# DeepGraphLearning/ULTRA

Hardware: AMD Instinct MI355X
Metric: triples scored/sec (all-tail ranking) on FB15k237 (higher is better)
Workload: dtype f32

## Files before the change

### include/ultra_nbfnet.h

```cpp
#ifndef ULTRA_NBFNET_H
#define ULTRA_NBFNET_H

#include <stdint.h>

#ifdef __cplusplus
extern "C" {
#endif

#define ULTRA_CONV_LAYER_NORM 1
#define ULTRA_CONV_RELU 2
#define ULTRA_CONV_RESIDUAL 4
#define ULTRA_LAYER0_MAX 8
#define ULTRA_LAYER0_ONLY_FILL 16
#define ULTRA_LAYER0_SKIP_FILL 32

int32_t ultra_conv_update(const void *x, const void *agg, const void *weight, const void *bias, const void *ln_weight,
                          const void *ln_bias, void *out, int64_t rows, int32_t input_dim, int32_t output_dim, float eps,
                          int32_t flags, void *stream);

int64_t ultra_conv_update_backward_workspace(int64_t rows);
int32_t ultra_conv_update_backward(const void *x, const void *agg, const void *grad_out, const void *weight, const void *bias,
                                   const void *ln_weight, const void *ln_bias, void *grad_x, void *grad_agg, void *grad_weight,
                                   void *grad_bias, void *grad_ln_weight, void *grad_ln_bias, void *workspace,
                                   int64_t workspace_bytes, int64_t rows, int32_t input_dim, int32_t output_dim, float eps,
                                   int32_t flags, void *stream);

int32_t ultra_readout(const void *hidden, const int64_t *t_index, const void *w1, const void *query, const void *b1,
                      const void *w2, const void *b2, const int32_t *order_dev, int64_t order_len, void *score, int64_t batch,
                      int64_t num_node, int64_t n_cand, int32_t hidden_dim, int32_t feature_dim, void *stream);

int32_t ultra_batch_prologue(const int64_t *triples, int64_t batch, int64_t n_cand, int64_t num_direct_rel, int64_t *h0,
                             int64_t *r0, int32_t *side, int32_t *valid, int64_t *rel_first, void *stream);
int32_t ultra_batch_prologue_rows(const int64_t *triples, int64_t batch, int64_t n_cand, int64_t num_direct_rel, int64_t *h0,
                                  int64_t *r0, int32_t *side, int32_t *valid, int64_t *rel_first, int64_t *cand, void *stream);
int32_t ultra_readout_batch(const void *hidden, const int64_t *triples, const int32_t *side, const void *w1, const void *query,
                            const void *b1, const void *w2, const void *b2, const int32_t *order_dev, int64_t order_len,
                            void *score, int64_t batch, int64_t num_node, int64_t n_cand, int32_t hidden_dim,
                            int32_t feature_dim, void *stream);

int32_t ultra_onehot_rows(void *out, const int64_t *rows, const void *values, int64_t batch, int64_t num_node, int64_t dim,
                          void *stream);

int32_t ultra_edge_keep_mask(const int64_t *head, const int64_t *tail, const int64_t *type, int64_t num_edge,
                             const int64_t *easy_key_sorted, int64_t n_easy, int64_t num_node, int64_t num_rel, void *keep,
                             void *stream);
int32_t ultra_easy_edge_keep(const int64_t *head, const int64_t *tail, const int64_t *type, int64_t num_edge, const int64_t *h,
                             const int64_t *t, const int64_t *r, int64_t n_triple, int64_t stride, int64_t num_node,
                             int64_t num_rel, int64_t inverse_offset, void *keep, void *stream);
int32_t ultra_leave_one_out_keep(const int64_t *head, const int64_t *tail, const int64_t *type, int64_t num_edge, const int64_t *h,
                                 const int64_t *t, const int64_t *r, int64_t n_sample, int64_t stride, int64_t num_node,
                                 int64_t num_rel, int64_t inverse_offset, void *keep, int64_t keep_stride, void *stream);
int64_t ultra_easy_edge_keep_table_workspace(int64_t n_triple);
int32_t ultra_easy_edge_keep_table(const int64_t *head, const int64_t *tail, const int64_t *type, int64_t num_edge,
                                   const int64_t *h, const int64_t *t, const int64_t *r, int64_t n_triple, int64_t stride,
                                   int64_t num_node, int64_t num_rel, int64_t inverse_offset, void *workspace,
                                   int64_t workspace_bytes, void *keep, void *stream);

int32_t ultra_query_boundary(void *out, void *query_out, const int64_t *rows, const void *table, const int64_t *pick,
                             int64_t batch, int64_t num_node, int64_t table_rows, int64_t dim, const void *w1, const void *b1,
                             void *qbias_out, void *stream);

int32_t ultra_relation_projection(const void *x, const void *w0, const void *b0, const void *w2, const void *b2, void *out,
                                  int64_t rows, int32_t n_layer, int32_t dim, void *stream);

int32_t ultra_relation_projection_layers(const void *x, const void *const *w0, const void *const *b0, const void *const *w2,
                                         const void *const *b2, void *out, int64_t rows, int32_t n_layer, int32_t dim, void *stream);

int64_t ultra_relation_projection_backward_workspace(int64_t rows, int32_t n_layer);
int32_t ultra_relation_projection_backward(const void *x, const void *const *w0, const void *const *b0, const void *const *w2,
                                           const void *const *grad_out, void *grad_x, void *grad_w0, void *grad_b0, void *grad_w2,
                                           void *grad_b2, void *workspace, int64_t workspace_bytes, int64_t rows, int32_t n_layer,
                                           int32_t dim, void *stream);

int32_t ultra_filtered_rank(const void *score, const int64_t *pos_index, const int64_t *known_ptr,
                            const int64_t *known_index, int64_t batch, int64_t n_cand, int64_t *rank_out,
                            int64_t *num_negative_out, void *stream);
int32_t ultra_filtered_rank_live(const void *score, const int64_t *pos_index, const int64_t *known_ptr,
                                 const int64_t *known_index, int64_t batch, int64_t n_cand, int64_t *rank_out,
                                 int64_t *num_negative_out, const int64_t *n_live, void *stream);

int32_t ultra_strict_negatives(const int64_t *sorted_keys_dev, int64_t n_key, const int64_t *anchor_dev, const int64_t *relation_dev,
                               const int64_t *positive_dev, const void *rand_dev, int64_t n_query, int64_t n_draw, int64_t num_node,
                               int64_t num_relation, int64_t *out_dev, void *stream);

int32_t ultra_ranking_loss(const void *pred, int64_t rows, int64_t n, float temperature, float uniform_weight, void *loss,
                           void *grad, void *stream);

int32_t ultra_readout_train_forward(const void *hid, const void *query, const void *w1, const void *b1, const void *w2,
                                    const void *b2, void *h, void *score, int64_t batch, int64_t n, void *stream);
int64_t ultra_readout_train_backward_workspace(int64_t batch, int64_t n);
int32_t ultra_readout_train_backward(const void *grad_score, const void *h, const void *hid, const void *query, const void *w1,
                                     const void *w2, void *grad_hid, void *grad_query, void *grad_w1, void *grad_b1, void *grad_w2,
                                     void *grad_b2, void *work, int64_t work_bytes, int64_t batch, int64_t n, void *stream);

int32_t ultra_relation_graph_bits(const int64_t *edge_index_dev, const int64_t *edge_type_dev, int64_t num_edge, int64_t num_node,
                                  int64_t num_relation, void *hbits_dev, void *tbits_dev, void *adj_dev, int64_t *row_counts_dev,
                                  void *stream);
int32_t ultra_relation_graph_emit(const void *adj_dev, const int64_t *row_offsets_dev, int64_t num_relation, int64_t total_edges,
                                  int64_t *edge_index_out_dev, int64_t *edge_type_out_dev, void *stream);
int32_t ultra_relation_graph_dense_adjacency(const void *adj_dev, int64_t num_relation, void *a_ex_out_dev, void *stream);
int32_t ultra_relation_graph_bits_keep(const int64_t *edge_index_dev, const int64_t *edge_type_dev, const float *keep_dev,
                                       int64_t num_edge, int64_t num_node, int64_t num_relation, void *hbits_dev, void *tbits_dev,
                                       void *adj_dev, int64_t *row_counts_dev, void *stream);
int32_t ultra_relation_graph_edge_keep(const void *adj_dev, int64_t num_relation, const int64_t *rel_edge_index_dev,
                                       const int64_t *rel_edge_type_dev, int64_t num_rel_edge, float *keep_out_dev, void *stream);
int32_t ultra_relation_graph_add_edges(const int64_t *edge_index_dev, const int64_t *edge_type_dev, int64_t num_edge, int64_t num_node,
                                       int64_t num_relation, void *hbits_dev, void *tbits_dev, void *adj_dev, int64_t *row_counts_dev,
                                       int32_t *changed_dev, void *stream);

#define ULTRA_BEAM_MAX 64
#define ULTRA_BEAM_HUB_DEGREE 256
int32_t ultra_beam_search_layer(const int64_t *row_ptr, const int32_t *csr_src, const int32_t *csr_type, const int32_t *csr_eid,
                                const int64_t *hub_rows, int64_t num_hub, int64_t num_node, int64_t num_edge,
                                const void *edge_grad, const void *dist_in, int64_t tail, int32_t num_beam, void *dist_out,
                                int64_t *back_edge_out, void *stream);

int32_t ultra_beam_search_layer_batch(const int64_t *row_ptr, const int32_t *csr_src, const int32_t *csr_type,
                                      const int32_t *csr_eid, const int64_t *hub_rows, int64_t num_hub, int64_t num_node,
                                      int64_t num_edge, int64_t num_sample, const void *edge_grad, const void *dist_in,
                                      const int64_t *tails, int32_t num_beam, void *dist_out, int64_t *back_edge_out,
                                      void *stream);

#define ULTRA_RANKING_LDS_ANSWERS 2048
int32_t ultra_symbolic_traversal(const int64_t *row_ptr, const int32_t *csr_src, const int32_t *csr_type, int64_t num_node,
                                 const int64_t *r_index, int64_t batch, int32_t dtype, const void *h, void *t, void *stream);
int32_t ultra_symbolic_traversal_keep(const int64_t *row_ptr, const int32_t *csr_src, const int32_t *csr_type,
                                      const float *keep_slot, int64_t num_node, const int64_t *r_index, int64_t batch, int32_t dtype,
                                      const void *h, void *t, void *stream);
int32_t ultra_answer_ranking(const void *pred, const uint8_t *keep, const int64_t *answers, const int64_t *ans_ptr,
                             const int64_t *hard_ptr, const int64_t *num_easy, const int64_t *ws_off, void *ws, int64_t batch,
                             int64_t num_node, int64_t *answer_ranking, int64_t *ranking, void *stream);

typedef struct {
    const int32_t *row_dev, *count_dev;
    const int32_t *add_ptr_dev, *add_src_dev, *add_type_dev;
    const int32_t *dead_ptr_dev, *dead_src_dev, *dead_type_dev;
    int64_t capacity_rows, capacity_edges, capacity_keys;
} ultra_traversal_edits;
int32_t ultra_symbolic_traversal_edit_rows(const int64_t *row_ptr, const int32_t *csr_src, const int32_t *csr_type,
                                           int64_t num_node, const ultra_traversal_edits *edits, const int64_t *r_index,
                                           int64_t batch, int32_t dtype, const void *h, void *t, void *stream);

int64_t ultra_traversal_dropout_mask_words(int64_t batch);
int32_t ultra_traversal_dropout(const int64_t *edge_index, const int64_t *edge_type, int64_t num_edge, int64_t num_node,
                                int64_t num_relation, int32_t inverse_rel_plus_one, const int32_t *deg_out, const int32_t *deg_in,
                                const int64_t *r_index, int64_t batch, int32_t dtype, const void *sym, const float *q,
                                const float *u1, const float *u2, float more_dropout, void *masks, float *keep, int32_t *k_out,
                                void *stream);
int32_t ultra_query_loss(const void *pred, const uint8_t *target, int64_t rows, int64_t n, float temperature, void *work,
                         void *loss, void *grad, void *stream);

#define ULTRA_TOPK_MAX 256
#define ULTRA_TOPK_CHUNK 4096
int64_t ultra_filtered_topk_workspace(int64_t batch, int64_t n_cand, int32_t k);
int32_t ultra_filtered_topk(const void *score, const int64_t *known_ptr, const int64_t *known_index, int64_t batch,
                            int64_t n_cand, int32_t k, int64_t *ids_out, void *scores_out, int64_t *count_out, void *workspace,
                            int64_t workspace_bytes, void *stream);
int32_t ultra_filtered_topk_live(const void *score, const int64_t *known_ptr, const int64_t *known_index, int64_t batch,
                                 int64_t n_cand, int32_t k, int64_t *ids_out, void *scores_out, int64_t *count_out,
                                 void *workspace, int64_t workspace_bytes, const int64_t *n_live, void *stream);

int32_t ultra_query_segment(const int32_t *entry_depth, const int32_t *push_row, const int32_t *pop_row, const int32_t *op_ptr,
                            const int32_t *ops, int64_t batch, int64_t num_node, int32_t stack_depth, int32_t dtype,
                            int32_t logic, void *stack, const void *push_src, int64_t push_rows, void *pop_dst,
                            int64_t pop_rows, void *sym_stack, const void *sym_push_src, void *sym_pop_dst, void *stream);
int32_t ultra_nonzero_lists(const void *x, int64_t batch, int64_t n, int64_t *counts, int64_t *ptr_out, int64_t *index_out,
                            int64_t capacity, void *stream);
int32_t ultra_nonzero_lists_live(const void *x, int64_t batch, int64_t n, int64_t *counts, int64_t *ptr_out,
                                 int64_t *index_out, int64_t capacity, const int64_t *n_live, void *stream);

int64_t ultra_filtered_above_workspace(int64_t batch, int64_t n_cand);
int32_t ultra_filtered_above(const void *score, const int64_t *known_ptr, const int64_t *known_index, int64_t batch,
                             int64_t n_cand, float threshold, int64_t *ptr_out, int64_t *ids_out, void *scores_out,
                             int64_t capacity, int64_t *size_out, void *workspace, int64_t workspace_bytes, void *stream);
int32_t ultra_filtered_above_live(const void *score, const int64_t *known_ptr, const int64_t *known_index, int64_t batch,
                                  int64_t n_cand, float threshold, int64_t *ptr_out, int64_t *ids_out, void *scores_out,
                                  int64_t capacity, int64_t *size_out, void *workspace, int64_t workspace_bytes,
                                  const int64_t *n_live, void *stream);

#ifdef __cplusplus
}
#endif
#endif
```

### ultra_amd/csrc/dense_kernels.hip

```cpp
#include <hip/hip_runtime.h>

#include <cstdint>
#include <cstdio>
#include <cstdlib>
#include <string>

#include "../../include/ultra_rspmm.h"
#include "plan.hpp"
#include "device_scope.hpp"
#include "torch_math.hpp"
#include "update_tile.hpp"

namespace ultra {

#ifndef ULTRA_CONV_DEBUG
#define ULTRA_CONV_DEBUG 0
#endif
constexpr int CONV_DBG_BITS = ULTRA_CONV_DEBUG ? CONV_DBG_NO_MATRIX : 0;

struct ConvParams {
    const float *x;
    const float *agg;
    const float *weight;
    const float *bias, *ln_w, *ln_b;
    float *out;
    long long rows;
    float eps;
    int flags;
};

__global__ void __launch_bounds__(512, 2) conv_update_kernel(const ConvParams p) {
    __shared__ __attribute__((aligned(16))) float lds_w[2 * 16 * 64 * 4];
    __shared__ float lds_vec[3 * 64];
    const int tid = threadIdx.x;
    for (int idx4 = tid; idx4 < 2 * 16 * 64; idx4 += blockDim.x) {
        const int l = idx4 & 63, i = (idx4 >> 6) & 15, m = idx4 >> 10;
        const float *wr = p.weight + (32 * m + (l & 31)) * 128 + 8 * i;
        const float4 w0 = *reinterpret_cast<const float4 *>(wr), w1 = *reinterpret_cast<const float4 *>(wr + 4);
        const bool odd = (l >> 5) != 0;
        reinterpret_cast<float4 *>(lds_w)[idx4] =
            make_float4(odd ? w0.y : w0.x, odd ? w1.y : w1.x, odd ? w0.w : w0.z, odd ? w1.w : w1.z);
    }
    if (tid < 64) {
        lds_vec[tid] = p.bias ? p.bias[tid] : 0.f;
        lds_vec[64 + tid] = (p.flags & CONV_LN) ? p.ln_w[tid] : 1.f;
        lds_vec[128 + tid] = (p.flags & CONV_LN) ? p.ln_b[tid] : 0.f;
    }
    __syncthreads();
    const int lane = tid & 63, wave = tid >> 6;
    const int j = lane & 31, h = lane >> 5;
    const float4 *w4 = reinterpret_cast<const float4 *>(lds_w);
    const long long ntile = (p.rows + 31) / 32;
    const int wpb = blockDim.x >> 6;
    const long long tstride = (long long)gridDim.x * wpb;
    long long tile = (long long)blockIdx.x * wpb + wave;
    float4 bx[8], ba[8];
    if (tile < ntile) {
        const long long r0 = tile * 32 + j;
        const long long rc0 = r0 < p.rows ? r0 : p.rows - 1;
        const float4 *xr = reinterpret_cast<const float4 *>(p.x + rc0 * 64);
        const float4 *ar = reinterpret_cast<const float4 *>(p.agg + rc0 * 64);
#pragma unroll
        for (int i = 0; i < 8; ++i) bx[i] = xr[2 * i + h];
#pragma unroll
        for (int i = 0; i < 8; ++i) ba[i] = ar[2 * i + h];
    }
    for (; tile < ntile; tile += tstride) {
        const long long row = tile * 32 + j;
        const bool valid = row < p.rows;
        float4 bxn[8], ban[8];
        {
            const long long tn = tile + tstride;
            const long long rn = (tn < ntile ? tn : tile) * 32 + j;
            const long long rcn = rn < p.rows ? rn : p.rows - 1;
            const float4 *xr = reinterpret_cast<const float4 *>(p.x + rcn * 64);
            const float4 *ar = reinterpret_cast<const float4 *>(p.agg + rcn * 64);
#pragma unroll
            for (int i = 0; i < 8; ++i) bxn[i] = xr[2 * i + h];
#pragma unroll
            for (int i = 0; i < 8; ++i) ban[i] = ar[2 * i + h];
        }
        f32x16 acc0, acc1;
#pragma unroll
        for (int r = 0; r < 16; ++r) {
            acc0[r] = 0.f;
            acc1[r] = 0.f;
        }
        float4 a0 = w4[(0 * 16 + 0) * 64 + lane];
        float4 a1 = w4[(1 * 16 + 0) * 64 + lane];
        float4 bs[16];
#pragma unroll
        for (int i = 0; i < 16; ++i) {
            bs[i] = i < 8 ? bx[i] : ba[i - 8];
            swap32(bs[i].x, bs[i].y);
            swap32(bs[i].z, bs[i].w);
        }
        __builtin_amdgcn_sched_barrier(0);
        if (!(p.flags & CONV_DBG_BITS & CONV_DBG_NO_MATRIX))
#pragma unroll
        for (int i = 0; i < 16; ++i) {
            const float4 b = bs[i];
            float4 a0n = a0, a1n = a1;
            if (i + 1 < 16) {
                a0n = w4[(0 * 16 + i + 1) * 64 + lane];
                a1n = w4[(1 * 16 + i + 1) * 64 + lane];
            }
            acc0 = __builtin_amdgcn_mfma_f32_32x32x2f32(a0.x, b.x, acc0, 0, 0, 0);
            acc1 = __builtin_amdgcn_mfma_f32_32x32x2f32(a1.x, b.x, acc1, 0, 0, 0);
            acc0 = __builtin_amdgcn_mfma_f32_32x32x2f32(a0.z, b.z, acc0, 0, 0, 0);
            acc1 = __builtin_amdgcn_mfma_f32_32x32x2f32(a1.z, b.z, acc1, 0, 0, 0);
            acc0 = __builtin_amdgcn_mfma_f32_32x32x2f32(a0.y, b.y, acc0, 0, 0, 0);
            acc1 = __builtin_amdgcn_mfma_f32_32x32x2f32(a1.y, b.y, acc1, 0, 0, 0);
            acc0 = __builtin_amdgcn_mfma_f32_32x32x2f32(a0.w, b.w, acc0, 0, 0, 0);
            acc1 = __builtin_amdgcn_mfma_f32_32x32x2f32(a1.w, b.w, acc1, 0, 0, 0);
            a0 = a0n;
            a1 = a1n;
            __builtin_amdgcn_sched_barrier(0);
        }
        float v[2][16];
#pragma unroll
        for (int r = 0; r < 16; ++r) {
            v[0][r] = acc0[r] + lds_vec[feat_of(0, r, h)];
            v[1][r] = acc1[r] + lds_vec[feat_of(1, r, h)];
        }
        if (p.flags & CONV_LN) {
            float mean, rstd;
            row_moments_pair(v, h, p.eps, mean, rstd);
#pragma unroll
            for (int m = 0; m < 2; ++m)
#pragma unroll
                for (int r = 0; r < 16; ++r) {
                    const int f = feat_of(m, r, h);
                    v[m][r] = ln_apply(v[m][r], mean, rstd, lds_vec[64 + f], lds_vec[128 + f]);
                }
        }
#pragma unroll
        for (int m = 0; m < 2; ++m)
#pragma unroll
            for (int g = 0; g < 4; ++g) {
                float4 y = make_float4(v[m][4 * g + 0], v[m][4 * g + 1], v[m][4 * g + 2], v[m][4 * g + 3]);
                if (p.flags & CONV_RELU) {
                    y.x = fmaxf(y.x, 0.f);
                    y.y = fmaxf(y.y, 0.f);
                    y.z = fmaxf(y.z, 0.f);
                    y.w = fmaxf(y.w, 0.f);
                }
                if (p.flags & CONV_RESIDUAL) {
                    const float4 xi = bx[4 * m + g];
                    y.x += xi.x;
                    y.y += xi.y;
                    y.z += xi.z;
                    y.w += xi.w;
                }
                if (valid) *reinterpret_cast<float4 *>(p.out + row * 64 + 32 * m + 8 * g + 4 * h) = y;
            }
#pragma unroll
        for (int i = 0; i < 8; ++i) {
            bx[i] = bxn[i];
            ba[i] = ban[i];
        }
    }
}

struct ReadoutParams {
    const float *hidden;
    const int64_t *t_index;
    const int64_t *triples;
    const int32_t *side;
    const float *w1;
    const float *query;
    const float *b1;
    const float *w2;
    const float *b2;
    const int32_t *order;
    int order_len;
    float *score;
    long long batch, num_node, n_cand;
};

constexpr int READOUT_ORDER_MAX = 640;
constexpr int READOUT_HID_STRIDE = 132;

__device__ __forceinline__ long long readout_node(const ReadoutParams &p, const long long row, const long long b, const long long c) {
    long long node = c;
    if (p.triples)
        node = p.triples[row * 3 + (p.side[b] ? 1 : 0)];
    else if (p.t_index)
        node = p.t_index[row];
    return (node >= 0 && node < p.num_node) ? node : -1;
}

__global__ void __launch_bounds__(512) readout_kernel(const ReadoutParams p) {
    __shared__ __attribute__((aligned(16))) float lds_w[4 * 16 * 64 * 4];
    __shared__ __attribute__((aligned(16))) float lds_hid[8][16 * READOUT_HID_STRIDE];
    __shared__ float lds_lane[8][16 * 16];
    __shared__ __attribute__((aligned(16))) float lds_w2[136], lds_b1[128];
    __shared__ __attribute__((aligned(16))) int lds_order[READOUT_ORDER_MAX];
    const int tid = threadIdx.x;
    for (int idx4 = tid; idx4 < 4 * 16 * 64; idx4 += blockDim.x) {
        const int l = idx4 & 63, i = (idx4 >> 6) & 15, m = idx4 >> 10;
        const float *wr = p.w1 + (32 * m + (l & 31)) * 128 + 8 * i;
        const float4 w0 = *reinterpret_cast<const float4 *>(wr), w1 = *reinterpret_cast<const float4 *>(wr + 4);
        const bool odd = (l >> 5) != 0;
        reinterpret_cast<float4 *>(lds_w)[idx4] =
            make_float4(odd ? w0.y : w0.x, odd ? w1.y : w1.x, odd ? w0.w : w0.z, odd ? w1.w : w1.z);
    }
    if (tid < 136) lds_w2[tid] = tid < 128 ? p.w2[tid] : 0.f;
    if (tid < 128) lds_b1[tid] = p.b1[tid];
    if (p.order) {
        for (int i = tid; i < p.order_len; i += blockDim.x) lds_order[i] = p.order[i];
    } else {
        for (int i = tid; i < 8 + 128; i += blockDim.x)
            lds_order[i] = i >= 8 ? i - 8 : (i == 0 || i == 1 ? 1 : (i == 3 ? 8 : (i == 4 ? 16 : 0)));
    }
    __syncthreads();
    const int lane = tid & 63, wave = tid >> 6;
    const int j = lane & 31, h = lane >> 5;
    const float4 *w4 = reinterpret_cast<const float4 *>(lds_w);
    float *hid = lds_hid[wave];
    float *lv = lds_lane[wave];
    const long long total = p.batch * p.n_cand;
    const long long ntile = (total + 31) / 32;
    const int wpb = blockDim.x >> 6;
    const auto load_tile = [&](const long long tile, float4 (&bh)[8], float4 (&bq)[8]) {
        const long long row = tile * 32 + j;
        const long long rowc = row < total ? row : total - 1;
        const long long b = rowc / p.n_cand;
        const long long c = rowc - b * p.n_cand;
        const long long node = readout_node(p, rowc, b, c) < 0 ? 0 : readout_node(p, rowc, b, c);
        const float4 *hr = reinterpret_cast<const float4 *>(p.hidden + (b * p.num_node + node) * 64);
#pragma unroll
        for (int i = 0; i < 8; ++i) bh[i] = hr[2 * i + h];
        const float *qr = p.query + b * 64 + h;
#pragma unroll
        for (int i = 0; i < 8; ++i) bq[i] = make_float4(qr[8 * i], qr[8 * i + 4], qr[8 * i + 2], qr[8 * i + 6]);
    };
    const long long tstride = (long long)gridDim.x * wpb;
    long long tile = (long long)blockIdx.x * wpb + wave;
    float4 bh[8], bq[8];
    if (tile < ntile) load_tile(tile, bh, bq);
    for (; tile < ntile; tile += tstride) {
        float4 bhn[8], bqn[8];
        load_tile(tile + tstride < ntile ? tile + tstride : tile, bhn, bqn);
        f32x16 acc[4];
#pragma unroll
        for (int m = 0; m < 4; ++m)
#pragma unroll
            for (int r = 0; r < 16; ++r) acc[m][r] = 0.f;
        float4 a[4];
#pragma unroll
        for (int m = 0; m < 4; ++m) a[m] = w4[(m * 16 + 0) * 64 + lane];
#pragma unroll
        for (int i = 0; i < 16; ++i) {
            float4 bb;
            if (i < 8) {
                bb = bh[i];
                swap32(bb.x, bb.y);
                swap32(bb.z, bb.w);
            } else {
                bb = bq[i - 8];
            }
            float4 an[4];
#pragma unroll
            for (int m = 0; m < 4; ++m) an[m] = (i + 1 < 16) ? w4[(m * 16 + i + 1) * 64 + lane] : a[m];
#pragma unroll
            for (int m = 0; m < 4; ++m) acc[m] = __builtin_amdgcn_mfma_f32_32x32x2f32(a[m].x, bb.x, acc[m], 0, 0, 0);
#pragma unroll
            for (int m = 0; m < 4; ++m) acc[m] = __builtin_amdgcn_mfma_f32_32x32x2f32(a[m].z, bb.z, acc[m], 0, 0, 0);
#pragma unroll
            for (int m = 0; m < 4; ++m) acc[m] = __builtin_amdgcn_mfma_f32_32x32x2f32(a[m].y, bb.y, acc[m], 0, 0, 0);
#pragma unroll
            for (int m = 0; m < 4; ++m) acc[m] = __builtin_amdgcn_mfma_f32_32x32x2f32(a[m].w, bb.w, acc[m], 0, 0, 0);
#pragma unroll
            for (int m = 0; m < 4; ++m) a[m] = an[m];
            __builtin_amdgcn_sched_barrier(0);
        }
#pragma unroll 1
        for (int pass = 0; pass < 2; ++pass) {
            if ((j >> 4) == pass) {
                const int jr = j & 15;
#pragma unroll
                for (int m = 0; m < 4; ++m)
#pragma unroll
                    for (int g = 0; g < 4; ++g) {
                        const int f = feat_of(m, 4 * g, h);
                        const float4 bb = *reinterpret_cast<const float4 *>(lds_b1 + f);
                        *reinterpret_cast<float4 *>(hid + jr * READOUT_HID_STRIDE + f) =
                            make_float4(fmaxf(acc[m][4 * g + 0] + bb.x, 0.f), fmaxf(acc[m][4 * g + 1] + bb.y, 0.f),
                                        fmaxf(acc[m][4 * g + 2] + bb.z, 0.f), fmaxf(acc[m][4 * g + 3] + bb.w, 0.f));
                    }
                if (h == 0) hid[jr * READOUT_HID_STRIDE + 128] = 0.f;
            }
            __builtin_amdgcn_fence(__ATOMIC_RELEASE, "wavefront");
            __builtin_amdgcn_wave_barrier();
            __builtin_amdgcn_fence(__ATOMIC_ACQUIRE, "wavefront");
            const int pr = lane & 15, sub = lane >> 4;
            const float *hrow = hid + pr * READOUT_HID_STRIDE;
            int hdr = 1;
            float s = 0.f;
            const int n_stage = lds_order[0];
            for (int st = 0; st < n_stage; ++st) {
                const int L = lds_order[hdr], carry = lds_order[hdr + 1];
                for (int q = sub; q < L; q += 4) {
                    const int off = lds_order[hdr + 2 + 2 * q], groups = lds_order[hdr + 3 + 2 * q];
                    float v = (q == 0 && carry) ? s : 0.f;
                    for (int g = 0; g < groups; ++g) {
                        const int4 w0 = *reinterpret_cast<const int4 *>(lds_order + off + 8 * g);
                        const int4 w1 = *reinterpret_cast<const int4 *>(lds_order + off + 8 * g + 4);
                        const int word[8] = {w0.x, w0.y, w0.z, w0.w, w1.x, w1.y, w1.z, w1.w};
                        float hv[8], wv[8];
#pragma unroll
                        for (int e = 0; e < 8; ++e) {
                            hv[e] = hrow[word[e] & 255];
                            wv[e] = lds_w2[word[e] & 255];
                        }
#pragma unroll
                        for (int e = 0; e < 8; ++e)
                            v = (word[e] & 256) ? v + hv[e] * wv[e] : __builtin_fmaf(hv[e], wv[e], v);
                    }
                    lv[q * 16 + pr] = v;
                }
                __builtin_amdgcn_fence(__ATOMIC_RELEASE, "wavefront");
                __builtin_amdgcn_wave_barrier();
                __builtin_amdgcn_fence(__ATOMIC_ACQUIRE, "wavefront");
                if (sub == 0) {
                    for (int half = L >> 1; half >= 1; half >>= 1)
                        for (int q = 0; q < half; ++q) lv[q * 16 + pr] = lv[q * 16 + pr] + lv[(q + half) * 16 + pr];
                    s = lv[pr];
                }
                hdr += 2 + 2 * L;
            }
            const long long prow = tile * 32 + 16 * pass + pr;
            if (sub == 0 && prow < total) {
                const long long pb = prow / p.n_cand;
                p.score[prow] = readout_node(p, prow, pb, prow - pb * p.n_cand) < 0 ? __builtin_nanf("") : s + p.b2[0];
            }
            __builtin_amdgcn_fence(__ATOMIC_RELEASE, "wavefront");
            __builtin_amdgcn_wave_barrier();
            __builtin_amdgcn_fence(__ATOMIC_ACQUIRE, "wavefront");
        }
#pragma unroll
        for (int i = 0; i < 8; ++i) {
            bh[i] = bhn[i];
            bq[i] = bqn[i];
        }
    }
}

constexpr int RELPROJ_MAX_LAYERS = 8;
struct RelProjParams {
    const float *x;
    const float *w0[RELPROJ_MAX_LAYERS], *b0[RELPROJ_MAX_LAYERS];
    const float *w2[RELPROJ_MAX_LAYERS], *b2[RELPROJ_MAX_LAYERS];
    float *out;
    long long rows;
    int n_layer;
};

constexpr int RELPROJ_TILES = 4;

__global__ void __launch_bounds__(256) relation_projection_kernel(const RelProjParams p) {
    constexpr int STRIDE = 68;
    __shared__ __attribute__((aligned(16))) float x_lds[RELPROJ_TILES][16 * STRIDE];
    __shared__ __attribute__((aligned(16))) float h_lds[RELPROJ_TILES][16 * STRIDE];
    using f32x4 = float __attribute__((ext_vector_type(4)));
    const int tid = threadIdx.x, lane = tid & 63, wave = tid >> 6;
    const int i16 = lane & 15, kk = lane >> 4;
    const int layer = blockIdx.y;
    const long long row_base = (long long)blockIdx.x * (16 * RELPROJ_TILES);
    const float *w0 = p.w0[layer], *w2 = p.w2[layer];
#pragma unroll
    for (int t = 0; t < RELPROJ_TILES; ++t) {
        const long long row = min(row_base + 16 * t + (tid >> 4), p.rows - 1);
        *reinterpret_cast<float4 *>(x_lds[t] + (tid >> 4) * STRIDE + 4 * (tid & 15)) =
            *reinterpret_cast<const float4 *>(p.x + row * 64 + 4 * (tid & 15));
    }
    float a0[16], a2[16];
    {
        const float4 *r0 = reinterpret_cast<const float4 *>(w0 + (16 * wave + i16) * 64);
        const float4 *r2 = reinterpret_cast<const float4 *>(w2 + (16 * wave + i16) * 64);
#pragma unroll
        for (int s = 0; s < 16; ++s) {
            const float4 v0 = r0[s], v2 = r2[s];
            a0[s] = kk == 0 ? v0.x : (kk == 1 ? v0.y : (kk == 2 ? v0.z : v0.w));
            a2[s] = kk == 0 ? v2.x : (kk == 1 ? v2.y : (kk == 2 ? v2.z : v2.w));
        }
    }
    const int f0 = 16 * wave + 4 * kk;
    float b0v[4], b2v[4];
#pragma unroll
    for (int r = 0; r < 4; ++r) {
        b0v[r] = p.b0[layer][f0 + r];
        b2v[r] = p.b2[layer][f0 + r];
    }
    __syncthreads();
    f32x4 d[RELPROJ_TILES];
#pragma unroll
    for (int t = 0; t < RELPROJ_TILES; ++t)
#pragma unroll
        for (int r = 0; r < 4; ++r) d[t][r] = 0.f;
#pragma unroll
    for (int s = 0; s < 16; ++s)
#pragma unroll
        for (int t = 0; t < RELPROJ_TILES; ++t)
            d[t] = __builtin_amdgcn_mfma_f32_16x16x4f32(a0[s], x_lds[t][i16 * STRIDE + 4 * s + kk], d[t], 0, 0, 0);
#pragma unroll
    for (int t = 0; t < RELPROJ_TILES; ++t)
#pragma unroll
        for (int r = 0; r < 4; ++r) h_lds[t][i16 * STRIDE + f0 + r] = fmaxf(d[t][r] + b0v[r], 0.f);
    __syncthreads();
#pragma unroll
    for (int t = 0; t < RELPROJ_TILES; ++t)
#pragma unroll
        for (int r = 0; r < 4; ++r) d[t][r] = 0.f;
#pragma unroll
    for (int s = 0; s < 16; ++s)
#pragma unroll
        for (int t = 0; t < RELPROJ_TILES; ++t)
            d[t] = __builtin_amdgcn_mfma_f32_16x16x4f32(a2[s], h_lds[t][i16 * STRIDE + 4 * s + kk], d[t], 0, 0, 0);
#pragma unroll
    for (int t = 0; t < RELPROJ_TILES; ++t) {
        const long long row = row_base + 16 * t + i16;
        if (row < p.rows)
            *reinterpret_cast<float4 *>(p.out + ((size_t)layer * p.rows + row) * 64 + f0) =
                make_float4(d[t][0] + b2v[0], d[t][1] + b2v[1], d[t][2] + b2v[2], d[t][3] + b2v[3]);
    }
}

static int grid_for(long long ntile, int waves_per_block, int blocks_per_cu = 2) {
    static int cu = 0;
    if (cu == 0) {
        int dev = 0, v = 0;
        cu = 256;
        if (hipGetDevice(&dev) == hipSuccess &&
            hipDeviceGetAttribute(&v, hipDeviceAttributeMultiprocessorCount, dev) == hipSuccess && v > 0)
            cu = v;
    }
    long long blocks = (ntile + waves_per_block - 1) / waves_per_block;
    const long long cap = (long long)cu * blocks_per_cu;
    if (blocks > cap) blocks = cap;
    if (blocks < 1) blocks = 1;
    return (int)blocks;
}

}

using namespace ultra;

extern "C" {

int32_t ultra_conv_update(const void *x, const void *agg, const void *weight, const void *bias, const void *ln_weight,
                          const void *ln_bias, void *out, int64_t rows, int32_t input_dim, int32_t output_dim, float eps,
                          int32_t flags, void *stream) {
    ULTRA_DEVICE_SCOPE(stream, x);
    if (input_dim != 64 || output_dim != 64) {
        set_error("ultra_conv_update: only input_dim = output_dim = 64 is built (the ULTRA checkpoints' shape)");
        return ULTRA_ERR_UNSUPPORTED;
    }
    if (!x || !agg || !weight || !out || rows < 0 || ((flags & CONV_LN) && (!ln_weight || !ln_bias))) {
        set_error("ultra_conv_update: NULL operand");
        return ULTRA_ERR_INVALID;
    }
    if (flags & ~(CONV_LN | CONV_RELU | CONV_RESIDUAL | CONV_DBG_BITS)) {
        set_error("ultra_conv_update: unknown flag bits " + std::to_string(flags & ~(CONV_LN | CONV_RELU | CONV_RESIDUAL | CONV_DBG_BITS)) +
                  " (CONV_DBG_NO_MATRIX exists only in a -DULTRA_CONV_DEBUG=1 build)");
        return ULTRA_ERR_INVALID;
    }
    if (rows == 0) return ULTRA_OK;
    ConvParams p;
    p.x = (const float *)x;
    p.agg = (const float *)agg;
    p.weight = (const float *)weight;
    p.bias = (const float *)bias;
    p.ln_w = (const float *)ln_weight;
    p.ln_b = (const float *)ln_bias;
    p.out = (float *)out;
    p.rows = rows;
    p.eps = eps;
    p.flags = flags;
    const long long ntile = (rows + 31) / 32;
    int threads = ntile >= 2048 ? 512 : 256;
    int grid = grid_for(ntile, threads / 64, threads == 512 ? 1 : 2);
    {
        static int env_threads = -1, env_grid = 0;
        if (env_threads < 0) {
            env_threads = 0;
            const char *env = std::getenv("ULTRA_CONV_GEOMETRY");
            if (env && std::sscanf(env, "%d,%d", &env_threads, &env_grid) != 2) env_threads = 0;
        }
        if (env_threads > 0 && env_grid > 0) threads = env_threads, grid = env_grid;
    }
    (void)hipGetLastError();
    hipLaunchKernelGGL(conv_update_kernel, dim3(grid), dim3(threads), 0, reinterpret_cast<hipStream_t>(stream), p);
    hipError_t e = hipGetLastError();
    if (e != hipSuccess) {
        set_error(std::string("conv_update_kernel launch: ") + hipGetErrorString(e));
        return ULTRA_ERR_HIP;
    }
    return ULTRA_OK;
}

static int launch_readout(ReadoutParams &p, const void *hidden, const void *w1, const void *query, const void *b1,
                          const void *w2, const void *b2, const int32_t *order, int64_t order_len, void *score, int64_t batch,
                          int64_t num_node, int64_t n_cand, int32_t hidden_dim, int32_t feature_dim, void *stream, const char *who) {
    if (hidden_dim != 64 || feature_dim != 128) {
        set_error(std::string(who) + ": only hidden_dim = 64, feature_dim = 128 is built (the ULTRA checkpoints' shape)");
        return ULTRA_ERR_UNSUPPORTED;
    }
    if (!hidden || !w1 || !query || !b1 || !w2 || !b2 || !score || batch < 0 || n_cand < 0) {
        set_error(std::string(who) + ": NULL operand");
        return ULTRA_ERR_INVALID;
    }
    if (order && (order_len < 5 || order_len > READOUT_ORDER_MAX)) {
        set_error(std::string(who) + ": summation program longer than 640 words (or empty)");
        return ULTRA_ERR_INVALID;
    }
    if (batch * n_cand == 0) return ULTRA_OK;
    p.hidden = (const float *)hidden;
    p.w1 = (const float *)w1;
    p.query = (const float *)query;
    p.b1 = (const float *)b1;
    p.w2 = (const float *)w2;
    p.b2 = (const float *)b2;
    p.order = order;
    p.order_len = (int)order_len;
    p.score = (float *)score;
    p.batch = batch;
    p.num_node = num_node;
    p.n_cand = n_cand;
    const long long ntile = (batch * n_cand + 31) / 32;
    const int grid = grid_for(ntile, 8, 1);
    (void)hipGetLastError();
    hipLaunchKernelGGL(readout_kernel, dim3(grid), dim3(512), 0, reinterpret_cast<hipStream_t>(stream), p);
    hipError_t e = hipGetLastError();
    if (e != hipSuccess) {
        set_error(std::string("readout_kernel launch: ") + hipGetErrorString(e));
        return ULTRA_ERR_HIP;
    }
    return ULTRA_OK;
}

int32_t ultra_readout(const void *hidden, const int64_t *t_index, const void *w1, const void *query, const void *b1,
                      const void *w2, const void *b2, const int32_t *order_dev, int64_t order_len, void *score, int64_t batch,
                      int64_t num_node, int64_t n_cand, int32_t hidden_dim, int32_t feature_dim, void *stream) {
    ULTRA_DEVICE_SCOPE(stream, hidden);
    ReadoutParams p;
    p.t_index = t_index;
    p.triples = nullptr;
    p.side = nullptr;
    return launch_readout(p, hidden, w1, query, b1, w2, b2, order_dev, order_len, score, batch, num_node, n_cand, hidden_dim,
                          feature_dim, stream, "ultra_readout");
}

int32_t ultra_readout_batch(const void *hidden, const int64_t *triples, const int32_t *side, const void *w1, const void *query,
                            const void *b1, const void *w2, const void *b2, const int32_t *order_dev, int64_t order_len,
                            void *score, int64_t batch, int64_t num_node, int64_t n_cand, int32_t hidden_dim,
                            int32_t feature_dim, void *stream) {
    ULTRA_DEVICE_SCOPE(stream, hidden);
    if (!triples || !side) {
        set_error("ultra_readout_batch: NULL operand");
        return ULTRA_ERR_INVALID;
    }
    ReadoutParams p;
    p.t_index = nullptr;
    p.triples = triples;
    p.side = side;
    return launch_readout(p, hidden, w1, query, b1, w2, b2, order_dev, order_len, score, batch, num_node, n_cand, hidden_dim,
                          feature_dim, stream, "ultra_readout_batch");
}

static int32_t launch_relation_projection(RelProjParams &p, void *stream) {
    const dim3 grid((unsigned)((p.rows + 16 * RELPROJ_TILES - 1) / (16 * RELPROJ_TILES)), (unsigned)p.n_layer);
    (void)hipGetLastError();
    hipLaunchKernelGGL(relation_projection_kernel, grid, dim3(256), 0, reinterpret_cast<hipStream_t>(stream), p);
    hipError_t e = hipGetLastError();
    if (e != hipSuccess) {
        set_error(std::string("relation_projection_kernel launch: ") + hipGetErrorString(e));
        return ULTRA_ERR_HIP;
    }
    return ULTRA_OK;
}

int32_t ultra_relation_projection(const void *x, const void *w0, const void *b0, const void *w2, const void *b2, void *out,
                                  int64_t rows, int32_t n_layer, int32_t dim, void *stream) {
    ULTRA_DEVICE_SCOPE(stream, x);
    if (dim != 64 || n_layer > RELPROJ_MAX_LAYERS) {
        set_error("ultra_relation_projection: only dim = 64 and at most 8 layers are built (the ULTRA checkpoints' shape)");
        return ULTRA_ERR_UNSUPPORTED;
    }
    if (!x || !w0 || !b0 || !w2 || !b2 || !out || rows < 0 || n_layer < 0) {
        set_error("ultra_relation_projection: NULL operand");
        return ULTRA_ERR_INVALID;
    }
    if (rows == 0 || n_layer == 0) return ULTRA_OK;
    RelProjParams p;
    p.x = (const float *)x;
    for (int l = 0; l < n_layer; ++l) {
        p.w0[l] = (const float *)w0 + (size_t)l * 64 * 64, p.b0[l] = (const float *)b0 + (size_t)l * 64;
        p.w2[l] = (const float *)w2 + (size_t)l * 64 * 64, p.b2[l] = (const float *)b2 + (size_t)l * 64;
    }
    p.out = (float *)out;
    p.rows = rows;
    p.n_layer = n_layer;
    return launch_relation_projection(p, stream);
}

int32_t ultra_relation_projection_layers(const void *x, const void *const *w0, const void *const *b0, const void *const *w2,
                                         const void *const *b2, void *out, int64_t rows, int32_t n_layer, int32_t dim,
                                         void *stream) {
    ULTRA_DEVICE_SCOPE(stream, x);
    if (dim != 64 || n_layer > RELPROJ_MAX_LAYERS) {
        set_error("ultra_relation_projection_layers: only dim = 64 and at most 8 layers are built (the ULTRA checkpoints' shape)");
        return ULTRA_ERR_UNSUPPORTED;
    }
    if (!x || !w0 || !b0 || !w2 || !b2 || !out || rows < 0 || n_layer < 0) {
        set_error("ultra_relation_projection_layers: NULL operand");
        return ULTRA_ERR_INVALID;
    }
    if (rows == 0 || n_layer == 0) return ULTRA_OK;
    RelProjParams p;
    p.x = (const float *)x;
    for (int l = 0; l < n_layer; ++l) {
        if (!w0[l] || !b0[l] || !w2[l] || !b2[l]) {
            set_error("ultra_relation_projection_layers: NULL layer parameter");
            return ULTRA_ERR_INVALID;
        }
        p.w0[l] = (const float *)w0[l], p.b0[l] = (const float *)b0[l], p.w2[l] = (const float *)w2[l], p.b2[l] = (const float *)b2[l];
    }
    p.out = (float *)out;
    p.rows = rows;
    p.n_layer = n_layer;
    return launch_relation_projection(p, stream);
}

}
```

Measured before the change: 212.5 million.

## Restructure readout kernel scheduling, prefetch, and precomputed walk coefficients with tracing hooks

Each wave now takes a contiguous range of tiles instead of a grid stride, and the first tile's hidden rows are prefetched before the weight staging so the global loads overlap setup. Two register buffers ping-pong between tiles, with incremental batch and candidate indices replacing per-tile divisions. The bias and ReLU move out of the per-pass store loop. The summation walk reads precomputed w2 coefficients and byte offsets, with a fast path when a group has no rounded elements. Invalid-node flags come from registers via shuffle instead of re-reading the triples. It also adds clock64 tracing and an env-var grid override, which cost only a pointer check when off, but the extra buffers raise register and LDS pressure.

```diff
diff --git a/include/ultra_nbfnet.h b/include/ultra_nbfnet.h
--- a/include/ultra_nbfnet.h
+++ b/include/ultra_nbfnet.h
@@ -37,6 +37,7 @@
                             const void *b1, const void *w2, const void *b2, const int32_t *order_dev, int64_t order_len,
                             void *score, int64_t batch, int64_t num_node, int64_t n_cand, int32_t hidden_dim,
                             int32_t feature_dim, void *stream);
+int32_t ultra_readout_trace(void *trace_dev);
 
 int32_t ultra_onehot_rows(void *out, const int64_t *rows, const void *values, int64_t batch, int64_t num_node, int64_t dim,
                           void *stream);
diff --git a/ultra_amd/csrc/dense_kernels.hip b/ultra_amd/csrc/dense_kernels.hip
--- a/ultra_amd/csrc/dense_kernels.hip
+++ b/ultra_amd/csrc/dense_kernels.hip
@@ -176,9 +176,11 @@
     int order_len;
     float *score;
     long long batch, num_node, n_cand;
+    long long *trace;
 };
 
 constexpr int READOUT_ORDER_MAX = 640;
+constexpr int READOUT_ELEM_OFFSET = 0x3fc, READOUT_ELEM_ROUNDED = 1 << 11, READOUT_ELEM_GROUP_ROUNDED = 1 << 12;
 constexpr int READOUT_HID_STRIDE = 132;
 
 __device__ __forceinline__ long long readout_node(const ReadoutParams &p, const long long row, const long long b, const long long c) {
@@ -194,54 +196,82 @@
     __shared__ __attribute__((aligned(16))) float lds_w[4 * 16 * 64 * 4];
     __shared__ __attribute__((aligned(16))) float lds_hid[8][16 * READOUT_HID_STRIDE];
     __shared__ float lds_lane[8][16 * 16];
-    __shared__ __attribute__((aligned(16))) float lds_w2[136], lds_b1[128];
+    __shared__ __attribute__((aligned(16))) float lds_w2p[READOUT_ORDER_MAX], lds_b1[128], lds_w2[136];
     __shared__ __attribute__((aligned(16))) int lds_order[READOUT_ORDER_MAX];
+    __shared__ __attribute__((aligned(16))) int lds_elem[READOUT_ORDER_MAX];
     const int tid = threadIdx.x;
-    for (int idx4 = tid; idx4 < 4 * 16 * 64; idx4 += blockDim.x) {
-        const int l = idx4 & 63, i = (idx4 >> 6) & 15, m = idx4 >> 10;
-        const float *wr = p.w1 + (32 * m + (l & 31)) * 128 + 8 * i;
-        const float4 w0 = *reinterpret_cast<const float4 *>(wr), w1 = *reinterpret_cast<const float4 *>(wr + 4);
-        const bool odd = (l >> 5) != 0;
-        reinterpret_cast<float4 *>(lds_w)[idx4] =
-            make_float4(odd ? w0.y : w0.x, odd ? w1.y : w1.x, odd ? w0.w : w0.z, odd ? w1.w : w1.z);
-    }
-    if (tid < 136) lds_w2[tid] = tid < 128 ? p.w2[tid] : 0.f;
-    if (tid < 128) lds_b1[tid] = p.b1[tid];
-    if (p.order) {
-        for (int i = tid; i < p.order_len; i += blockDim.x) lds_order[i] = p.order[i];
-    } else {
-        for (int i = tid; i < 8 + 128; i += blockDim.x)
-            lds_order[i] = i >= 8 ? i - 8 : (i == 0 || i == 1 ? 1 : (i == 3 ? 8 : (i == 4 ? 16 : 0)));
-    }
-    __syncthreads();
     const int lane = tid & 63, wave = tid >> 6;
     const int j = lane & 31, h = lane >> 5;
+    long long *tr = (p.trace && tid == 0) ? p.trace + 16 * blockIdx.x : nullptr;
+    long long t_mat = 0, t_epi = 0, t_walk = 0, n_done = 0, t0 = 0;
+    if (tr) tr[0] = clock64();
+    const long long total = p.batch * p.n_cand;
+    const long long ntile = (total + 31) / 32;
+    const long long nwave = (long long)gridDim.x * (blockDim.x >> 6), gwave = (long long)blockIdx.x * (blockDim.x >> 6) + wave;
+    const long long per_wave = ntile / nwave, longer = ntile - per_wave * nwave;
+    long long tile = gwave * per_wave + (gwave < longer ? gwave : longer);
+    const long long tend = tile + per_wave + (gwave < longer ? 1 : 0);
+    long long row_n = tile * 32 + j, b_n = 0, c_n = 0;
+    if (tile < tend) {
+        b_n = row_n / p.n_cand;
+        c_n = row_n - b_n * p.n_cand;
+    }
+    const auto load_next = [&](float4 (&bh)[8], const float *&qr, int &bad) {
+        const bool in = row_n < total;
+        const long long rowc = in ? row_n : total - 1, b = in ? b_n : p.batch - 1, c = in ? c_n : p.n_cand - 1;
+        const long long id = readout_node(p, rowc, b, c);
+        bad = id < 0;
+        const long long node = id < 0 ? 0 : id;
+        const float4 *hr = reinterpret_cast<const float4 *>(p.hidden + (b * p.num_node + node) * 64);
+#pragma unroll
+        for (int i = 0; i < 8; ++i) bh[i] = hr[2 * i + h];
+        qr = p.query + b * 64 + h;
+        row_n += 32;
+        c_n += 32;
+        while (c_n >= p.n_cand) c_n -= p.n_cand, ++b_n;
+    };
+    float4 bh0[8], bh1[8];
+    const float *qr0 = p.query, *qr1 = p.query;
+    int bad0 = 0, bad1 = 0;
+    if (tile < tend) load_next(bh0, qr0, bad0);
+    for (int s = 0; s < 8; ++s) {
+        const int g = wave * 8 + s;
+        const int row = (g >> 2) * 8 + (j >> 2), i = (g & 3) * 4 + (j & 3);
+        float4 v = *reinterpret_cast<const float4 *>(p.w1 + row * 128 + 8 * i + 4 * h);
+        swap32(v.x, v.y);
+        swap32(v.z, v.w);
+        reinterpret_cast<float4 *>(lds_w)[((row >> 5) * 16 + i) * 64 + (row & 31) + 32 * h] = v;
+    }
+    if (tid < 128) lds_b1[tid] = p.b1[tid];
+    if (tid < 136) lds_w2[tid] = tid < 128 ? p.w2[tid] : 0.f;
+    const int n_word = p.order ? p.order_len : 8 + 128;
+    for (int i = tid; i < n_word; i += blockDim.x)
+        lds_order[i] = p.order ? p.order[i] : (i >= 8 ? i - 8 : (i == 0 || i == 1 ? 1 : (i == 3 ? 8 : (i == 4 ? 16 : 0))));
+    __syncthreads();
+    for (int i = tid; i < n_word; i += blockDim.x) {
+        const int w = lds_order[i], k = w & 255;
+        lds_w2p[i] = lds_w2[k < 136 ? k : 128];
+        int group = 0;
+        if ((i & 3) == 0)
+            for (int e = 0; e < 8 && i + e < n_word; ++e) group |= lds_order[i + e] & 256;
+        lds_elem[i] = (k << 2) | ((w & 256) ? READOUT_ELEM_ROUNDED : 0) | (group ? READOUT_ELEM_GROUP_ROUNDED : 0);
+    }
+    __syncthreads();
+    if (tr) tr[1] = clock64();
     const float4 *w4 = reinterpret_cast<const float4 *>(lds_w);
     float *hid = lds_hid[wave];
     float *lv = lds_lane[wave];
-    const long long total = p.batch * p.n_cand;
-    const long long ntile = (total + 31) / 32;
-    const int wpb = blockDim.x >> 6;
-    const auto load_tile = [&](const long long tile, float4 (&bh)[8], float4 (&bq)[8]) {
-        const long long row = tile * 32 + j;
-        const long long rowc = row < total ? row : total - 1;
-        const long long b = rowc / p.n_cand;
-        const long long c = rowc - b * p.n_cand;
-        const long long node = readout_node(p, rowc, b, c) < 0 ? 0 : readout_node(p, rowc, b, c);
-        const float4 *hr = reinterpret_cast<const float4 *>(p.hidden + (b * p.num_node + node) * 64);
-#pragma unroll
-        for (int i = 0; i < 8; ++i) bh[i] = hr[2 * i + h];
-        const float *qr = p.query + b * 64 + h;
+    if (p.trace) {
+        asm volatile("s_waitcnt vmcnt(0)" ::: "memory");
+        if (tr) tr[2] = clock64();
+    }
+    float4 bq[8];
+    const auto load_query = [&](const float *qr) {
 #pragma unroll
         for (int i = 0; i < 8; ++i) bq[i] = make_float4(qr[8 * i], qr[8 * i + 4], qr[8 * i + 2], qr[8 * i + 6]);
     };
-    const long long tstride = (long long)gridDim.x * wpb;
-    long long tile = (long long)blockIdx.x * wpb + wave;
-    float4 bh[8], bq[8];
-    if (tile < ntile) load_tile(tile, bh, bq);
-    for (; tile < ntile; tile += tstride) {
-        float4 bhn[8], bqn[8];
-        load_tile(tile + tstride < ntile ? tile + tstride : tile, bhn, bqn);
+    const auto do_tile = [&](const long long tile, const float4 (&bh)[8], const int bad) {
+        if (tr) t0 = clock64();
         f32x16 acc[4];
 #pragma unroll
         for (int m = 0; m < 4; ++m)
@@ -275,6 +305,20 @@
             for (int m = 0; m < 4; ++m) a[m] = an[m];
             __builtin_amdgcn_sched_barrier(0);
         }
+        if (tr) {
+            const long long t = clock64();
+            t_mat += t - t0, t0 = t, ++n_done;
+        }
+#pragma unroll
+        for (int m = 0; m < 4; ++m)
+#pragma unroll
+            for (int g = 0; g < 4; ++g) {
+                const float4 bb = *reinterpret_cast<const float4 *>(lds_b1 + feat_of(m, 4 * g, h));
+                acc[m][4 * g + 0] = fmaxf(acc[m][4 * g + 0] + bb.x, 0.f);
+                acc[m][4 * g + 1] = fmaxf(acc[m][4 * g + 1] + bb.y, 0.f);
+                acc[m][4 * g + 2] = fmaxf(acc[m][4 * g + 2] + bb.z, 0.f);
+                acc[m][4 * g + 3] = fmaxf(acc[m][4 * g + 3] + bb.w, 0.f);
+            }
 #pragma unroll 1
         for (int pass = 0; pass < 2; ++pass) {
             if ((j >> 4) == pass) {
@@ -282,20 +326,20 @@
 #pragma unroll
                 for (int m = 0; m < 4; ++m)
 #pragma unroll
-                    for (int g = 0; g < 4; ++g) {
-                        const int f = feat_of(m, 4 * g, h);
-                        const float4 bb = *reinterpret_cast<const float4 *>(lds_b1 + f);
-                        *reinterpret_cast<float4 *>(hid + jr * READOUT_HID_STRIDE + f) =
-                            make_float4(fmaxf(acc[m][4 * g + 0] + bb.x, 0.f), fmaxf(acc[m][4 * g + 1] + bb.y, 0.f),
-                                        fmaxf(acc[m][4 * g + 2] + bb.z, 0.f), fmaxf(acc[m][4 * g + 3] + bb.w, 0.f));
-                    }
+                    for (int g = 0; g < 4; ++g)
+                        *reinterpret_cast<float4 *>(hid + jr * READOUT_HID_STRIDE + feat_of(m, 4 * g, h)) =
+                            make_float4(acc[m][4 * g + 0], acc[m][4 * g + 1], acc[m][4 * g + 2], acc[m][4 * g + 3]);
                 if (h == 0) hid[jr * READOUT_HID_STRIDE + 128] = 0.f;
             }
             __builtin_amdgcn_fence(__ATOMIC_RELEASE, "wavefront");
             __builtin_amdgcn_wave_barrier();
             __builtin_amdgcn_fence(__ATOMIC_ACQUIRE, "wavefront");
+            if (tr) {
+                const long long t = clock64();
+                t_epi += t - t0, t0 = t;
+            }
             const int pr = lane & 15, sub = lane >> 4;
-            const float *hrow = hid + pr * READOUT_HID_STRIDE;
+            const char *hrow_b = reinterpret_cast<const char *>(hid + pr * READOUT_HID_STRIDE);
             int hdr = 1;
             float s = 0.f;
             const int n_stage = lds_order[0];
@@ -305,18 +349,28 @@
                     const int off = lds_order[hdr + 2 + 2 * q], groups = lds_order[hdr + 3 + 2 * q];
                     float v = (q == 0 && carry) ? s : 0.f;
                     for (int g = 0; g < groups; ++g) {
-                        const int4 w0 = *reinterpret_cast<const int4 *>(lds_order + off + 8 * g);
-                        const int4 w1 = *reinterpret_cast<const int4 *>(lds_order + off + 8 * g + 4);
+                        const int4 w0 = *reinterpret_cast<const int4 *>(lds_elem + off + 8 * g);
+                        const int4 w1 = *reinterpret_cast<const int4 *>(lds_elem + off + 8 * g + 4);
+                        const float4 c0 = *reinterpret_cast<const float4 *>(lds_w2p + off + 8 * g);
+                        const float4 c1 = *reinterpret_cast<const float4 *>(lds_w2p + off + 8 * g + 4);
                         const int word[8] = {w0.x, w0.y, w0.z, w0.w, w1.x, w1.y, w1.z, w1.w};
-                        float hv[8], wv[8];
-#pragma unroll
-                        for (int e = 0; e < 8; ++e) {
-                            hv[e] = hrow[word[e] & 255];
-                            wv[e] = lds_w2[word[e] & 255];
+                        const float wv[8] = {c0.x, c0.y, c0.z, c0.w, c1.x, c1.y, c1.z, c1.w};
+                        float hv[8];
+                        if (__builtin_amdgcn_ballot_w64((w0.x & READOUT_ELEM_GROUP_ROUNDED) != 0) == 0) {
+#pragma unroll
+                            for (int e = 0; e < 8; ++e)
+                                hv[e] = *reinterpret_cast<const float *>(
+                                    hrow_b + ((e & 3) == 0 ? (word[e] & READOUT_ELEM_OFFSET) : word[e]));
+#pragma unroll
+                            for (int e = 0; e < 8; ++e) v = __builtin_fmaf(hv[e], wv[e], v);
+                        } else {
+#pragma unroll
+                            for (int e = 0; e < 8; ++e)
+                                hv[e] = *reinterpret_cast<const float *>(hrow_b + (word[e] & READOUT_ELEM_OFFSET));
+#pragma unroll
+                            for (int e = 0; e < 8; ++e)
+                                v = (word[e] & READOUT_ELEM_ROUNDED) ? v + hv[e] * wv[e] : __builtin_fmaf(hv[e], wv[e], v);
                         }
-#pragma unroll
-                        for (int e = 0; e < 8; ++e)
-                            v = (word[e] & 256) ? v + hv[e] * wv[e] : __builtin_fmaf(hv[e], wv[e], v);
                     }
                     lv[q * 16 + pr] = v;
                 }
@@ -331,19 +385,31 @@
                 hdr += 2 + 2 * L;
             }
             const long long prow = tile * 32 + 16 * pass + pr;
-            if (sub == 0 && prow < total) {
-                const long long pb = prow / p.n_cand;
-                p.score[prow] = readout_node(p, prow, pb, prow - pb * p.n_cand) < 0 ? __builtin_nanf("") : s + p.b2[0];
-            }
+            const int prow_bad = __shfl(bad, 16 * pass + pr);
+            if (sub == 0 && prow < total) p.score[prow] = prow_bad ? __builtin_nanf("") : s + p.b2[0];
             __builtin_amdgcn_fence(__ATOMIC_RELEASE, "wavefront");
             __builtin_amdgcn_wave_barrier();
             __builtin_amdgcn_fence(__ATOMIC_ACQUIRE, "wavefront");
-        }
-#pragma unroll
-        for (int i = 0; i < 8; ++i) {
-            bh[i] = bhn[i];
-            bq[i] = bqn[i];
-        }
+            if (tr) {
+                const long long t = clock64();
+                t_walk += t - t0, t0 = t;
+            }
+        }
+    };
+    while (tile < tend) {
+        load_query(qr0);
+        if (tile + 1 < tend) load_next(bh1, qr1, bad1);
+        do_tile(tile, bh0, bad0);
+        if (++tile >= tend) break;
+        load_query(qr1);
+        if (tile + 1 < tend) load_next(bh0, qr0, bad0);
+        do_tile(tile, bh1, bad1);
+        ++tile;
+    }
+    if (p.trace && lane == 0) {
+        const long long t = clock64();
+        p.trace[16 * blockIdx.x + 8 + wave] = t;
+        if (tr) tr[3] = t_mat, tr[4] = t_epi, tr[5] = t_walk, tr[6] = t, tr[7] = n_done;
     }
 }
 
@@ -500,6 +566,8 @@
     return ULTRA_OK;
 }
 
+static thread_local long long *g_readout_trace = nullptr;
+
 static int launch_readout(ReadoutParams &p, const void *hidden, const void *w1, const void *query, const void *b1,
                           const void *w2, const void *b2, const int32_t *order, int64_t order_len, void *score, int64_t batch,
                           int64_t num_node, int64_t n_cand, int32_t hidden_dim, int32_t feature_dim, void *stream, const char *who) {
@@ -528,8 +596,13 @@
     p.batch = batch;
     p.num_node = num_node;
     p.n_cand = n_cand;
+    p.trace = g_readout_trace;
     const long long ntile = (batch * n_cand + 31) / 32;
-    const int grid = grid_for(ntile, 8, 1);
+    int grid = grid_for(ntile, 8, 1);
+    if (const char *env = std::getenv("ULTRA_READOUT_GRID")) {
+        const long long n = std::atoll(env), most = (ntile + 7) / 8;
+        if (n > 0) grid = (int)(n < most ? n : most);
+    }
     (void)hipGetLastError();
     hipLaunchKernelGGL(readout_kernel, dim3(grid), dim3(512), 0, reinterpret_cast<hipStream_t>(stream), p);
     hipError_t e = hipGetLastError();
@@ -569,6 +642,11 @@
                           feature_dim, stream, "ultra_readout_batch");
 }
 
+int32_t ultra_readout_trace(void *trace_dev) {
+    g_readout_trace = static_cast<long long *>(trace_dev);
+    return ULTRA_OK;
+}
+
 static int32_t launch_relation_projection(RelProjParams &p, void *stream) {
     const dim3 grid((unsigned)((p.rows + 16 * RELPROJ_TILES - 1) / (16 * RELPROJ_TILES)), (unsigned)p.n_layer);
     (void)hipGetLastError();
```

After: 215.6 million (median of 3 runs). About the same (+1.5%).
